# lipku/LiveTalking

Hardware: NVIDIA H100
Metric: lip-sync frames/sec (wav2lip256, 256x256, batch 16, mel + U-Net fwd + paste-back) (higher is better)
Workload: dtype f16 (fp32 accumulate); mel f64; paste u8

## Files before the change

### livetalking_b200/csrc/conv_halo.cu

```cuda
#include <cuda.h>

#include <atomic>
#include <mutex>
#include <utility>

#include "conv_halo.h"
#include "ltb_internal.h"
#include "ptx_sm90.cuh"

#ifdef LTB_HALO_DIAG
#include <cstdlib>
#define LTB_DIAG(bit) (p.dbg & (bit))
#else
#define LTB_DIAG(bit) 0
#endif

namespace ltb {

constexpr int kHaloP = 10;
constexpr int kHaloThreads = 384;
constexpr int kProducerRegs = 40, kConsumerRegs = 232;
constexpr int kSms = 132;

template <int BN, int NSUB, int NACC, int TAPS, int RC = 0>
// ... 478 lines not shown
          const size_t opix = halo_pix(img, ty, tx, q >> 1, 0, wq * 16 + (lane >> 2) + 8 * (q & 1), row_ok);
          if (q < 2 * NSUB && row_ok) {
            float ha0 = head_sw[96], ha1 = head_sw[97], ha2 = head_sw[98];
#pragma unroll
            for (int i = 0; i < 4; ++i)
#pragma unroll
              for (int src = 0; src < 4; ++src) {
                const float2 f = __half22float2(*reinterpret_cast<__half2*>(&hv[src][i]));
                const int cc = 8 * i + 2 * src;
                ha0 = fmaf(f.x, head_sw[cc], ha0);
                ha0 = fmaf(f.y, head_sw[cc + 1], ha0);
                ha1 = fmaf(f.x, head_sw[32 + cc], ha1);
                ha1 = fmaf(f.y, head_sw[32 + cc + 1], ha1);
                ha2 = fmaf(f.x, head_sw[64 + cc], ha2);
                ha2 = fmaf(f.y, head_sw[64 + cc + 1], ha2);
              }
            float* o = p.head_out + opix * 3;
            o[0] = (1.f / (1.f + expf(-ha0))) * 255.f;
            o[1] = (1.f / (1.f + expf(-ha1))) * 255.f;
            o[2] = (1.f / (1.f + expf(-ha2))) * 255.f;
          }
        }
      }
    }
  }

  __syncthreads();
  if (gn_smem) {
    for (int i = tid; i < p.gn_images * p.gn_groups * 2; i += kHaloThreads) {
      const float v = gn_acc[i];
      if (v != 0.f) atomicAdd(p.gn_stats + i, v);
    }
  }
}

typedef CUresult (*EncodeTiledFn)(CUtensorMap*, CUtensorMapDataType, cuuint32_t, void*, const cuuint64_t*, const cuuint64_t*,
                                  const cuuint32_t*, const cuuint32_t*, CUtensorMapInterleave, CUtensorMapSwizzle,
                                  CUtensorMapL2promotion, CUtensorMapFloatOOBfill);

static EncodeTiledFn get_encode() {
  static EncodeTiledFn fn = nullptr;
  static std::once_flag once;
  std::call_once(once, []() {
    void* p = nullptr;
    cudaDriverEntryPointQueryResult q;
    if (cudaGetDriverEntryPoint("cuTensorMapEncodeTiled", &p, cudaEnableDefault, &q) == cudaSuccess &&
        q == cudaDriverEntryPointSuccess)
      fn = reinterpret_cast<EncodeTiledFn>(p);
  });
  return fn;
}

bool encode_tmap_f16(CUtensorMap* tm, int rank, const void* base, const cuuint64_t* dims, const cuuint64_t* strides_bytes,
                     const cuuint32_t* box, int spatial_stride) {
  EncodeTiledFn fn = get_encode();
  if (!fn) return false;
  cuuint32_t es[5] = {1, (cuuint32_t)spatial_stride, (cuuint32_t)spatial_stride, 1, 1};
  return fn(tm, CU_TENSOR_MAP_DATA_TYPE_FLOAT16, (cuuint32_t)rank, const_cast<void*>(base), dims, strides_bytes, box, es,
            CU_TENSOR_MAP_INTERLEAVE_NONE, CU_TENSOR_MAP_SWIZZLE_128B, CU_TENSOR_MAP_L2_PROMOTION_L2_256B,
            CU_TENSOR_MAP_FLOAT_OOB_FILL_NONE) == CUDA_SUCCESS;
}

static bool is_conv3x3(const ConvParams& p) {
  if (p.nphases != 1 || p.ph[0].ntaps != 9 || p.sy != 1 || p.sx != 1 || p.osy != 1 || p.osx != 1) return false;
  for (int t = 0; t < 9; ++t)
    if (p.ph[0].dy[t] != t / 3 - 1 || p.ph[0].dx[t] != t % 3 - 1) return false;
  return p.IH == p.GH && p.IW == p.GW && p.OH == p.GH && p.OW == p.GW;
}
static bool is_convT(const ConvParams& p) {
  if (p.nphases != 4 || p.osy != 2 || p.osx != 2 || p.sy != 1 || p.sx != 1) return false;
  const int nt[4] = {1, 2, 2, 4};
  for (int i = 0; i < 4; ++i)
    if (p.ph[i].ntaps != nt[i]) return false;
  return p.IH == p.GH && p.IW == p.GW && p.OH == 2 * p.GH && p.OW == 2 * p.GW;
}

static bool is_conv3x3_s2(const ConvParams& p) {
  if (p.nphases != 1 || p.ph[0].ntaps != 9 || p.sy != 2 || p.sx != 2 || p.osy != 1 || p.osx != 1) return false;
  for (int t = 0; t < 9; ++t)
    if (p.ph[0].dy[t] != t / 3 - 1 || p.ph[0].dx[t] != t % 3 - 1) return false;
  return p.IH == 2 * p.GH && p.IW == 2 * p.GW && p.OH == p.GH && p.OW == p.GW;
}

static bool is_upconv(const ConvParams& p) {
  return p.upconv == 1 && p.nphases == 4 && p.osy == 2 && p.osx == 2 && p.sy == 1 && p.sx == 1 && p.IH == p.GH && p.IW == p.GW &&
         p.OH == 2 * p.GH && p.OW == 2 * p.GW;
}

static bool is_gemm(const ConvParams& p) {
  return p.nphases == 1 && p.ph[0].ntaps == 1 && p.ph[0].dy[0] == 0 && p.ph[0].dx[0] == 0 && p.sy == 1 && p.sx == 1 && p.osy == 1 &&
         p.osx == 1 && p.IH == p.GH && p.IW == p.GW && p.OH == p.GH && p.OW == p.GW;
}

static bool pick_cfg(const ConvParams& p, int* BN, int* NSUB, int* NACC);

bool conv_halo_supported(const ConvParams& p) {
  if (p.zbatch > 1) return false;
  if ((p.OCtot % 8) || (p.oc_off % 8) || (reinterpret_cast<uintptr_t>(p.out) % 16)) return false;
  if (p.res && ((p.RCtot % 8) || (p.rc_off % 8) || (reinterpret_cast<uintptr_t>(p.res) % 16))) return false;
  if (p.group_slot && (!is_gemm(p) || (p.w_slot_stride * 2) % 16 != 0)) return false;
  if (is_gemm(p)) {
    return p.Cout % 32 == 0 && p.Cin % 8 == 0 && p.Cin >= 32 && (p.ICtot % 8) == 0 && (p.ic_off % 8) == 0 && (p.Ktot % 8) == 0 &&
           (p.ph[0].koff % 8) == 0 && p.M >= 512 && get_encode() != nullptr;
  }
  if (is_conv3x3_s2(p)) {
    return p.Cout % 32 == 0 && p.Cin >= 64 && (p.ICtot % 8) == 0 && (p.ic_off % 8) == 0 && p.Ktot == 9 * p.Cin && p.GH >= 16 &&
           p.GW >= 8 && get_encode() != nullptr;
  }
  if (is_upconv(p))
    return p.Cout % 64 == 0 && p.Cin >= 16 && (p.ICtot % 8) == 0 && (p.ic_off % 8) == 0 && p.Ktot == 16 * p.Cin && get_encode() != nullptr;
  if (!(is_conv3x3(p) || is_convT(p))) return false;
  if (p.Cout % 32 != 0 || p.Cin < 16) return false;
// ... 288 lines not shown
```

### livetalking_b200/csrc/conv_halo.h

```cpp
#pragma once
#include <cuda.h>
#include <cuda_runtime.h>

#include <cstring>

#include "conv_params.h"

namespace ltb {

struct alignas(64) HaloParams {
  CUtensorMap tm_in;
  CUtensorMap tm_w;
  __half* out;
  const __half* res;
  const float* bias;
  int N, M, Cin;
  int OCtot, oc_off, RCtot, rc_off;
  int OH, OW, osy, osx;
  int GH, GW;
  int relu;
  int res_halo;
  int halo_y0, halo_x0;
  int acc_oy[4], acc_ox[4];
  int tiles_x, tiles_y, tiles_n, total_tiles;
  float* gn_stats;
  int gn_groups, gn_cpg, gn_hw, gn_images;
  const float* head_w;
  const float* head_b;
  float* head_out;
  const int* group_slot;
  int group_rows, group_tiles;
  long long bias_slot_stride;
#ifdef LTB_HALO_DIAG
  int dbg;
#endif
};

struct HaloPlan {
  HaloParams hp;
  int BN, NSUB, NACC, TAPS;
  bool grouped;
};

bool conv_halo_supported(const ConvParams& p);
int conv_halo_make_plan(const ConvParams& p, const __half* w_tap_major, HaloPlan* out);
cudaError_t launch_conv_halo(const HaloPlan& pl, cudaStream_t st);
bool encode_tmap_f16(CUtensorMap* tm, int rank, const void* base, const cuuint64_t* dims, const cuuint64_t* strides_bytes,
                     const cuuint32_t* box, int spatial_stride = 1);
int conv_halo_sms();
int conv_halo_resident_chunks(const HaloPlan& pl, int sms);
bool conv_halo_gn_fusable(const HaloPlan& pl, int cout_total, int groups, int hw);
cudaError_t launch_w_tap_major(const __half* w, __half* wt, int cout, int cin, cudaStream_t st, int ntaps = 9);
cudaError_t launch_w_tap_major_convT(const __half* w, __half* wt, int cout, int cin, cudaStream_t st);

}
```

### livetalking_b200/csrc/conv_plan.cu

```cuda
#include <cstring>
#include <string>
#include <vector>

#include "../../include/ltb200.h"
#include "conv_plan.h"
#include "ltb_internal.h"

namespace ltb {

static const int kTd[2][2] = {{0, 0}, {0, 1}};
static const int kTk[2][2] = {{1, 0}, {2, 0}};
static const int kTn[2] = {1, 2};
static const int kUd[2][2] = {{-1, 0}, {0, 1}};

ConvParams conv_params(ConvMode mode, int N, ConvSlice in, int IH, int IW, int Cin, ConvSlice out, int OH, int OW, int Cout,
                       ConvSlice res, const __half* w, int Ktot, int w_koff, const float* bias, bool relu, ConvTaps taps) {
  ConvParams p;
  std::memset(&p, 0, sizeof(p));
  p.in = in.p;
  p.N = N;
  p.IH = IH;
  p.IW = IW;
  p.ICtot = in.Ctot;
  p.ic_off = in.off;
// ... 9 lines not shown
  p.res = res.p;
  p.RCtot = res.Ctot;
  p.rc_off = res.off;
  p.w = w;
  p.Ktot = Ktot;
  p.bias = bias;
  p.relu = relu ? 1 : 0;
  if (mode == ConvMode::Dense) {
    p.sy = taps.sy;
    p.sx = taps.sx;
    p.GH = OH;
    p.GW = OW;
    p.nphases = 1;
    ConvPhase& ph = p.ph[0];
    ph.ntaps = taps.KH * taps.KW;
    ph.koff = w_koff;
    for (int kh = 0; kh < taps.KH; ++kh)
      for (int kw = 0; kw < taps.KW; ++kw) {
        ph.dy[kh * taps.KW + kw] = (signed char)(kh - taps.pad_t);
        ph.dx[kh * taps.KW + kw] = (signed char)(kw - taps.pad_l);
      }
  } else {
    const bool up = mode == ConvMode::Upsample2x;
    p.GH = IH;
    p.GW = IW;
    p.osy = p.osx = 2;
    p.nphases = 4;
    p.upconv = up ? 1 : 0;
    int koff = w_koff;
    for (int a = 0; a < 2; ++a)
      for (int b = 0; b < 2; ++b) {
        ConvPhase& ph = p.ph[a * 2 + b];
        const int na = up ? 2 : kTn[a], nb = up ? 2 : kTn[b];
        ph.ntaps = na * nb;
        ph.koff = koff;
        ph.ooy = a;
        ph.oox = b;
        for (int i = 0; i < na; ++i)
          for (int j = 0; j < nb; ++j) {
            ph.dy[i * nb + j] = (signed char)(up ? kUd[a][i] : kTd[a][i]);
            ph.dx[i * nb + j] = (signed char)(up ? kUd[b][j] : kTd[b][j]);
          }
        koff += ph.ntaps * Cin;
      }
  }
  p.M = N * p.GH * p.GW;
  return p;
}

int conv_plan(const ConvParams& p, const __half* w_tap, ConvPath path, ConvPlan* out) {
  out->p = p;
  out->halo = false;
  out->pingpong = false;
  if (p.group_slot) {
    if (p.group_images < 1 || p.N % p.group_images || p.slots < 1 || p.w_slot_stride < 0 || p.bias_slot_stride < 0)
      return LTB_FAIL("conv: grouped weights need N divisible by group_images >= 1, slots >= 1 and non-negative slot strides");
    if (p.zbatch > 1 || p.upconv) return LTB_FAIL("conv: grouped weights cannot be combined with zbatch or the fused upsample");
  }
  if (path == ConvPath::Gather) return 0;
  if (w_tap && conv_pingpong_supported(p)) {
    if (conv_pingpong_make_plan(p, w_tap, &out->pp) != 0) return LTB_FAIL("conv: ping-pong plan / tensor map creation failed");
    out->pingpong = true;
    return 0;
  }
  const bool gemm = p.nphases == 1 && p.ph[0].ntaps == 1;
  if (!((w_tap || gemm) && conv_halo_supported(p))) {
    if (path == ConvPath::Auto) return 0;
    return LTB_FAIL("conv: the halo kernel cannot run " + std::to_string(p.N) + "x" + std::to_string(p.IH) + "x" + std::to_string(p.IW) +
                    "x" + std::to_string(p.Cin) + " -> " + std::to_string(p.OH) + "x" + std::to_string(p.OW) + "x" + std::to_string(p.Cout) +
                    (w_tap || gemm ? "" : " without tap-major weights"));
  }
  if (conv_halo_make_plan(p, w_tap, &out->hp) != 0) return LTB_FAIL("conv: halo plan / tensor map creation failed");
  out->halo = true;
  return 0;
}

cudaError_t conv_launch(const ConvPlan& pl, cudaStream_t st, float* splitk_ws, size_t ws_floats) {
  if (pl.pingpong) return launch_conv_pingpong(pl.pp, st);
  return pl.halo ? launch_conv_halo(pl.hp, st) : launch_conv_gather(pl.p, st, splitk_ws, ws_floats);
}

bool conv_plan_variant(const ConvPlan& pl, bool have_ws, size_t ws_floats, ltb_conv_variant* out) {
  std::memset(out, 0, sizeof(*out));
  out->grouped = pl.p.group_slot != nullptr;
  if (pl.pingpong) {
    out->kernel = 2;
    out->taps = 9;
    out->bn = 64;
    out->nsub = 1;
    out->nacc = 1;
    out->resident_chunks = 1;
    out->res_halo = 1;
    return true;
  }
  if (pl.halo) {
    out->kernel = 1;
    out->taps = pl.hp.TAPS;
    out->bn = pl.hp.BN;
    out->nsub = pl.hp.NSUB;
    out->nacc = pl.hp.NACC;
    out->resident_chunks = conv_halo_resident_chunks(pl.hp, conv_halo_sms());
    out->res_halo = pl.hp.hp.res_halo;
    return true;
  }
  int ksplit = 0;
  if (!conv_gather_pick(pl.p, have_ws, ws_floats, &out->bn, &out->kb, &ksplit)) return false;
  out->ksplit = ksplit > 1 ? ksplit : 1;
  return true;
}

bool conv_plan_fuse_gn_stats(ConvPlan* pl, float* stats, int groups, int hw) {
  const ConvParams& p = pl->p;
  if (!pl->halo || pl->hp.grouped || p.oc_off != 0 || p.OCtot != p.Cout || !conv_halo_gn_fusable(pl->hp, p.Cout, groups, hw)) return false;
  HaloParams& h = pl->hp.hp;
  h.gn_stats = stats;
  h.gn_groups = groups;
  h.gn_cpg = p.Cout / groups;
  h.gn_hw = hw;
  h.gn_images = p.M / hw;
  return true;
}

bool conv_plan_fuse_head(ConvPlan* pl, const float* w, const float* b, float* out) {
  if (!pl->halo || pl->hp.grouped || pl->hp.BN != 32 || pl->p.Cout != 32) return false;
  pl->hp.hp.head_w = w;
  pl->hp.hp.head_b = b;
  pl->hp.hp.head_out = out;
  return true;
}

static void pack_conv_w(const float* w, int cout, int cin, int KH, int KW, std::vector<__half>& out) {
  out.resize((size_t)cout * KH * KW * cin);
  for (int co = 0; co < cout; ++co)
    for (int kh = 0; kh < KH; ++kh)
      for (int kw = 0; kw < KW; ++kw)
        for (int ci = 0; ci < cin; ++ci)
          out[((size_t)co * KH * KW + kh * KW + kw) * cin + ci] = __float2half(w[(((size_t)co * cin + ci) * KH + kh) * KW + kw]);
}
static void pack_convT_w(const float* w, int cin, int cout, std::vector<__half>& out) {
  out.resize((size_t)cout * 9 * cin);
  for (int co = 0; co < cout; ++co) {
    size_t k = 0;
    for (int a = 0; a < 2; ++a)
      for (int b = 0; b < 2; ++b)
        for (int i = 0; i < kTn[a]; ++i)
          for (int j = 0; j < kTn[b]; ++j) {
            const int kh = kTk[a][i], kw = kTk[b][j];
            for (int ci = 0; ci < cin; ++ci, ++k)
              out[(size_t)co * 9 * cin + k] = __float2half(w[(((size_t)ci * cout + co) * 3 + kh) * 3 + kw]);
          }
  }
}

}

using namespace ltb;

static int conv2d_f16_impl(const ltb_conv_desc* d, const void* in_f16, const float* w_f32, const float* bias_f32,
                           const void* res_f16, void* out_f16, int reps, float* ms_out) {
  if (!d || !in_f16 || !w_f32 || !bias_f32 || !out_f16) return LTB_FAIL("null argument");
  if (d->has_res && !res_f16) return LTB_FAIL("has_res set but res is null");
  int OH, OW, Ktot;
  std::vector<__half> wp;
  if (d->transposed) {
    if (d->KH != 3 || d->KW != 3) return LTB_FAIL("transposed conv: only k=3,s=2,p=1,op=1");
    OH = d->IH * 2;
    OW = d->IW * 2;
    Ktot = 9 * d->Cin;
    pack_convT_w(w_f32, d->Cin, d->Cout, wp);
  } else {
    if (d->KH * d->KW > kMaxTaps) return LTB_FAIL("kernel too large");
    OH = conv_out_dim(d->IH, d->KH, d->sy, d->pad);
    OW = conv_out_dim(d->IW, d->KW, d->sx, d->pad);
    Ktot = d->KH * d->KW * d->Cin;
    pack_conv_w(w_f32, d->Cout, d->Cin, d->KH, d->KW, wp);
  }
  if (OH <= 0 || OW <= 0) return LTB_FAIL("empty output");
  const size_t in_b = (size_t)d->N * d->IH * d->IW * d->Cin * 2, out_b = (size_t)d->N * OH * OW * d->Cout * 2;
  __half *din = nullptr, *dout = nullptr, *dw = nullptr, *dres = nullptr, *dwt = nullptr;
  float* dbias = nullptr;
  float* dws = nullptr;
  cudaEvent_t e0 = nullptr, e1 = nullptr;
  int rc = 0;
  auto cleanup = [&]() {
    cudaFree(din);
    cudaFree(dout);
    cudaFree(dw);
    cudaFree(dres);
    cudaFree(dwt);
    cudaFree(dws);
    cudaFree(dbias);
    if (e0) cudaEventDestroy(e0);
    if (e1) cudaEventDestroy(e1);
  };
#define CK(x)                                                             \
  do {                                                                    \
    cudaError_t _e = (x);                                                 \
    if (_e != cudaSuccess) {                                              \
      rc = LTB_FAIL(std::string(#x) + ": " + cudaGetErrorString(_e));     \
      cleanup();                                                          \
      return rc;                                                          \
    }                                                                     \
  } while (0)
  CK(cudaMalloc(&din, in_b));
  CK(cudaMalloc(&dout, out_b));
  CK(cudaMalloc(&dw, wp.size() * 2));
  CK(cudaMalloc(&dbias, (size_t)d->Cout * 4));
  CK(cudaMemcpy(din, in_f16, in_b, cudaMemcpyHostToDevice));
  CK(cudaMemcpy(dw, wp.data(), wp.size() * 2, cudaMemcpyHostToDevice));
  CK(cudaMemcpy(dbias, bias_f32, (size_t)d->Cout * 4, cudaMemcpyHostToDevice));
  CK(cudaMemset(dout, 0xFF, out_b));
  if (d->has_res) {
    CK(cudaMalloc(&dres, out_b));
    CK(cudaMemcpy(dres, res_f16, out_b, cudaMemcpyHostToDevice));
  }
  if (d->KH == 3 && d->KW == 3) {
    CK(cudaMalloc(&dwt, wp.size() * 2));
    CK(d->transposed ? launch_w_tap_major_convT(dw, dwt, d->Cout, d->Cin, nullptr) : launch_w_tap_major(dw, dwt, d->Cout, d->Cin, nullptr));
  }
  const ConvParams p = conv_params(d->transposed ? ConvMode::Transposed : ConvMode::Dense, d->N, {din, d->Cin, 0}, d->IH, d->IW, d->Cin,
                                   {dout, d->Cout, 0}, OH, OW, d->Cout, d->has_res ? ConvSlice{dres, d->Cout, 0} : ConvSlice{}, dw, Ktot, 0,
                                   dbias, d->relu != 0, {d->KH, d->KW, d->sy, d->sx, d->pad, d->pad});
  const ConvPath path = d->force_path == 1 ? ConvPath::Gather : d->force_path == 2 ? ConvPath::Halo : ConvPath::Auto;
  ConvPlan pl;
  if (conv_plan(p, dwt, path, &pl)) {
    cleanup();
    return 1;
  }
  const size_t ws_floats = (pl.halo || pl.pingpong) ? 0 : (size_t)1 << 22;
  if (ws_floats) {
    CK(cudaMalloc(&dws, ws_floats * sizeof(float)));
    CK(cudaMemset(dws, 0, ws_floats * sizeof(float)));
  }
  CK(conv_launch(pl, nullptr, dws, ws_floats));
  if (reps > 0) {
    CK(cudaEventCreate(&e0));
    CK(cudaEventCreate(&e1));
    for (int i = 0; i < 3; ++i) CK(conv_launch(pl, nullptr, dws, ws_floats));
    CK(cudaEventRecord(e0, nullptr));
    for (int i = 0; i < reps; ++i) CK(conv_launch(pl, nullptr, dws, ws_floats));
    CK(cudaEventRecord(e1, nullptr));
    CK(cudaEventSynchronize(e1));
    CK(cudaEventElapsedTime(ms_out, e0, e1));
    *ms_out /= reps;
  }
  CK(cudaDeviceSynchronize());
  CK(cudaMemcpy(out_f16, dout, out_b, cudaMemcpyDeviceToHost));
#undef CK
  cleanup();
  return 0;
}

extern "C" {

int ltb_conv2d_f16(const ltb_conv_desc* d, const void* in_f16, const float* w_f32, const float* bias_f32,
                   const void* res_f16, void* out_f16) {
  return conv2d_f16_impl(d, in_f16, w_f32, bias_f32, res_f16, out_f16, 0, nullptr);
}

int ltb_conv2d_f16_timed(const ltb_conv_desc* d, const void* in_f16, const float* w_f32, const float* bias_f32,
                         const void* res_f16, void* out_f16, int reps, float* ms_per_launch) {
  if (reps < 1 || !ms_per_launch) return LTB_FAIL("conv2d_f16_timed: reps >= 1 and a result pointer are required");
  return conv2d_f16_impl(d, in_f16, w_f32, bias_f32, res_f16, out_f16, reps, ms_per_launch);
}

}
```

### livetalking_b200/csrc/conv_plan.h

```cpp
#pragma once
#include <cuda_runtime.h>

#include "conv_halo.h"
#include "conv_pingpong.h"

struct ltb_conv_variant;

namespace ltb {

struct ConvSlice {
  const __half* p;
  int Ctot, off;
};

enum class ConvMode {
  Dense,
  Transposed,
  Upsample2x,
};
struct ConvTaps {
  int KH, KW, sy, sx, pad_t, pad_l;
};

inline int conv_out_dim(int in, int k, int s, int pad) { return (in + 2 * pad - k) / s + 1; }

ConvParams conv_params(ConvMode mode, int N, ConvSlice in, int IH, int IW, int Cin, ConvSlice out, int OH, int OW, int Cout,
                       ConvSlice res, const __half* w, int Ktot, int w_koff, const float* bias, bool relu, ConvTaps taps = {});

enum class ConvPath {
  Auto,
  Gather,
  Halo,
};
struct ConvPlan {
  ConvParams p{};
  bool halo = false;
  HaloPlan hp{};
  bool pingpong = false;
  PingpongParams pp{};
};

int conv_plan(const ConvParams& p, const __half* w_tap, ConvPath path, ConvPlan* out);
cudaError_t conv_launch(const ConvPlan& pl, cudaStream_t st, float* splitk_ws, size_t ws_floats);
bool conv_plan_variant(const ConvPlan& pl, bool have_ws, size_t ws_floats, ltb_conv_variant* out);

bool conv_plan_fuse_gn_stats(ConvPlan* pl, float* stats, int groups, int hw);
bool conv_plan_fuse_head(ConvPlan* pl, const float* w, const float* b, float* out);

}
```

### livetalking_b200/csrc/ptx_sm90.cuh

```cuda
#pragma once
#include <cuda_fp16.h>
#include <cstdint>
#include <cstdio>

namespace ltb {

__device__ __forceinline__ uint32_t smem_u32(const void* p) {
  return static_cast<uint32_t>(__cvta_generic_to_shared(p));
}

__device__ __forceinline__ void mbar_init(uint32_t bar, uint32_t count) {
  asm volatile("mbarrier.init.shared::cta.b64 [%0], %1;" ::"r"(bar), "r"(count) : "memory");
}
__device__ __forceinline__ void mbar_fence_init() {
  asm volatile("fence.mbarrier_init.release.cluster;" ::: "memory");
}
__device__ __forceinline__ void mbar_arrive(uint32_t bar) {
  asm volatile("mbarrier.arrive.shared::cta.b64 _, [%0];" ::"r"(bar) : "memory");
}
__device__ __forceinline__ void mbar_arrive_expect_tx(uint32_t bar, uint32_t bytes) {
  asm volatile("mbarrier.arrive.expect_tx.shared::cta.b64 _, [%0], %1;" ::"r"(bar), "r"(bytes) : "memory");
}
__device__ __forceinline__ bool mbar_try_wait(uint32_t bar, uint32_t parity) {
  uint32_t ok;
// ... 62 lines not shown
      "l"(tmap), "r"(bar), "r"(c0), "r"(c1), "r"(c2), "r"(c3), "r"(c4)
      : "memory");
}

__device__ __forceinline__ void ldmatrix_x4(uint32_t& r0, uint32_t& r1, uint32_t& r2, uint32_t& r3, uint32_t saddr) {
  asm volatile("ldmatrix.sync.aligned.m8n8.x4.shared.b16 {%0, %1, %2, %3}, [%4];"
               : "=r"(r0), "=r"(r1), "=r"(r2), "=r"(r3)
               : "r"(saddr)
               : "memory");
}

__device__ __forceinline__ void ldmatrix_x4_trans(uint32_t& r0, uint32_t& r1, uint32_t& r2, uint32_t& r3, uint32_t saddr) {
  asm volatile("ldmatrix.sync.aligned.m8n8.x4.trans.shared.b16 {%0, %1, %2, %3}, [%4];"
               : "=r"(r0), "=r"(r1), "=r"(r2), "=r"(r3)
               : "r"(saddr)
               : "memory");
}
__device__ __forceinline__ void stmatrix_x4_trans(uint32_t saddr, uint32_t r0, uint32_t r1, uint32_t r2, uint32_t r3) {
  asm volatile("stmatrix.sync.aligned.m8n8.x4.trans.shared.b16 [%0], {%1, %2, %3, %4};" ::"r"(saddr), "r"(r0), "r"(r1), "r"(r2), "r"(r3)
               : "memory");
}

__device__ __forceinline__ void tma_store_4d(const void* tmap, uint32_t src, int c0, int c1, int c2, int c3) {
  asm volatile("cp.async.bulk.tensor.4d.global.shared::cta.bulk_group [%0, {%2, %3, %4, %5}], [%1];" ::"l"(tmap), "r"(src), "r"(c0),
               "r"(c1), "r"(c2), "r"(c3)
               : "memory");
}
__device__ __forceinline__ void bulk_commit() { asm volatile("cp.async.bulk.commit_group;" ::: "memory"); }
template <int N>
__device__ __forceinline__ void bulk_wait_read() {
  asm volatile("cp.async.bulk.wait_group.read %0;" ::"n"(N) : "memory");
}
template <int N>
__device__ __forceinline__ void bulk_wait() {
  asm volatile("cp.async.bulk.wait_group %0;" ::"n"(N) : "memory");
}

__device__ __forceinline__ void named_sync(uint32_t id, uint32_t threads) {
  asm volatile("bar.sync %0, %1;" ::"r"(id), "r"(threads) : "memory");
}
__device__ __forceinline__ void named_arrive(uint32_t id, uint32_t threads) {
  asm volatile("bar.arrive %0, %1;" ::"r"(id), "r"(threads) : "memory");
}

__device__ __forceinline__ uint64_t wgmma_desc(uint32_t saddr, uint32_t lbo_bytes, uint32_t sbo_bytes, uint32_t layout) {
  uint64_t d = 0;
  d |= (uint64_t)((saddr & 0x3FFFF) >> 4);
  d |= (uint64_t)((lbo_bytes >> 4) & 0x3FFF) << 16;
  d |= (uint64_t)((sbo_bytes >> 4) & 0x3FFF) << 32;
  d |= (uint64_t)(layout & 3) << 62;
  return d;
}
__host__ __device__ constexpr uint32_t wgmma_hi_128b(uint32_t sbo_bytes) { return (sbo_bytes >> 4) | (1u << 30); }
__device__ __forceinline__ uint32_t wgmma_lo(uint32_t saddr) { return ((saddr & 0x3FFFFu) >> 4) | (1u << 16); }
__device__ __forceinline__ uint64_t wgmma_lohi(uint32_t lo, uint32_t hi) { return ((uint64_t)hi << 32) | lo; }

__device__ __forceinline__ void wgmma_fence() { asm volatile("wgmma.fence.sync.aligned;" ::: "memory"); }
__device__ __forceinline__ void wgmma_commit() { asm volatile("wgmma.commit_group.sync.aligned;" ::: "memory"); }
template <int N>
__device__ __forceinline__ void wgmma_wait() {
  asm volatile("wgmma.wait_group.sync.aligned %0;" ::"n"(N) : "memory");
}
template <int R>
__device__ __forceinline__ void wgmma_fence_regs(float (&d)[R]) {
#pragma unroll
  for (int i = 0; i < R; ++i) asm volatile("" : "+f"(d[i])::"memory");
}

template <int N>
struct Wgmma;
#define LTB_D1(i) "+f"(d[i])
#define LTB_D2(i) LTB_D1(i), LTB_D1(i + 1)
#define LTB_D4(i) LTB_D2(i), LTB_D2(i + 2)
#define LTB_D8(i) LTB_D4(i), LTB_D4(i + 4)
#define LTB_D16(i) LTB_D8(i), LTB_D8(i + 8)
#define LTB_D32(i) LTB_D16(i), LTB_D16(i + 16)
#define LTB_D64(i) LTB_D32(i), LTB_D32(i + 32)
#define LTB_D128(i) LTB_D64(i), LTB_D64(i + 64)
#define LTB_WG_HEAD(P) "{\n.reg .pred p;\nsetp.ne.b32 p, %" P ", 0;\nwgmma.mma_async.sync.aligned.m64n"
#define LTB_WG_SS(N, REGS, A, B, P) LTB_WG_HEAD(P) N "k16.f32.f16.f16 " REGS ", %" A ", %" B ", p, 1, 1, 0, 0;\n}\n"
#define LTB_WG_RS(N, REGS, A, B, P) \
  LTB_WG_HEAD(P) N "k16.f32.f16.f16 " REGS ", {%" A "}, %" B ", p, 1, 1, 0;\n}\n"

template <>
struct Wgmma<16> {
#define LTB_R "{%0,%1,%2,%3,%4,%5,%6,%7}"
  __device__ __forceinline__ static void ss(float (&d)[8], uint64_t a, uint64_t b, uint32_t acc) {
    asm volatile(LTB_WG_SS("16", LTB_R, "8", "9", "10") : LTB_D8(0) : "l"(a), "l"(b), "r"(acc));
  }
  __device__ __forceinline__ static void rs(float (&d)[8], const uint32_t (&a)[4], uint64_t b, uint32_t acc) {
    asm volatile(LTB_WG_RS("16", LTB_R, "8,%9,%10,%11", "12", "13") : LTB_D8(0)
                 : "r"(a[0]), "r"(a[1]), "r"(a[2]), "r"(a[3]), "l"(b), "r"(acc));
  }
#undef LTB_R
};

template <>
struct Wgmma<32> {
#define LTB_R "{%0,%1,%2,%3,%4,%5,%6,%7,%8,%9,%10,%11,%12,%13,%14,%15}"
  __device__ __forceinline__ static void ss(float (&d)[16], uint64_t a, uint64_t b, uint32_t acc) {
    asm volatile(LTB_WG_SS("32", LTB_R, "16", "17", "18") : LTB_D16(0) : "l"(a), "l"(b), "r"(acc));
  }
  __device__ __forceinline__ static void rs(float (&d)[16], const uint32_t (&a)[4], uint64_t b, uint32_t acc) {
    asm volatile(LTB_WG_RS("32", LTB_R, "16,%17,%18,%19", "20", "21") : LTB_D16(0)
                 : "r"(a[0]), "r"(a[1]), "r"(a[2]), "r"(a[3]), "l"(b), "r"(acc));
  }
// ... 151 lines not shown
```

### livetalking_b200/csrc/w2l_engine.cu

```cuda
#include <cstring>
#include <memory>
#include <mutex>
#include <string>
#include <vector>

#include "../../include/ltb200.h"
#include "conv_plan.h"
#include "ltb_internal.h"
#include "stem_umma.h"

namespace ltb {

static thread_local std::string g_last_error;
void set_error(const std::string& msg) { g_last_error = msg; }

bool pdl_default() {
  static const bool on = [] {
    const char* e = std::getenv("LTB_NO_PDL");
    return !(e && e[0] && e[0] != '0');
  }();
  return on;
}
static thread_local int g_pdl = -1;
bool pdl_enabled() { return g_pdl < 0 ? pdl_default() : g_pdl == 1; }
// ... 240 lines not shown
  const int catS[8] = {512, 512, 512, 256, 128, 64, 32, 16};
  __half* cat[8];
  for (int i = 0; i < 8; ++i) {
    void* p;
    if (dev_alloc(s, (size_t)B * catH[i] * catH[i] * (catD[i] + catS[i]) * 2, &p, true)) return 1;
    cat[i] = static_cast<__half*>(p);
  }
  const size_t tmp_bytes = (size_t)B * 256 * 256 * 64 * 2;
  __half* ring[2] = {nullptr, nullptr};
  int ring_next = 0;
  auto new_tmp = [&](int H, int W, int C, View* v) -> int {
    void* p = nullptr;
    if (keep) {
      if (dev_alloc(s, (size_t)B * H * W * C * 2, &p, true)) return 1;
    } else {
      if (!ring[ring_next]) {
        if (dev_alloc(s, tmp_bytes, &p, true)) return 1;
        ring[ring_next] = static_cast<__half*>(p);
      }
      p = ring[ring_next];
      ring_next ^= 1;
    }
    *v = View{static_cast<__half*>(p), H, W, C, 0, C};
    return 0;
  };
  __half* aring[2] = {nullptr, nullptr};
  int aring_next = 0;
  auto new_atmp = [&](int H, int W, int C, View* v) -> int {
    void* p = nullptr;
    if (keep) {
      if (dev_alloc(s, (size_t)B * H * W * C * 2, &p, true)) return 1;
    } else {
      if (!aring[aring_next]) {
        if (dev_alloc(s, (size_t)B * 80 * 16 * 32 * 2, &p, true)) return 1;
        aring[aring_next] = static_cast<__half*>(p);
      }
      p = aring[aring_next];
      aring_next ^= 1;
    }
    *v = View{static_cast<__half*>(p), H, W, C, 0, C};
    return 0;
  };
  auto cat_dec = [&](int i) { return View{cat[i], catH[i], catH[i], catD[i] + catS[i], 0, catD[i]}; };
  auto cat_skip = [&](int i) { return View{cat[i], catH[i], catH[i], catD[i] + catS[i], catD[i], catS[i]}; };
  auto cat_all = [&](int i) { return View{cat[i], catH[i], catH[i], catD[i] + catS[i], 0, catD[i] + catS[i]}; };

  auto record = [&](int li, const View& v) {
    s->louts[li] = LayerOut{v.p, v.H, v.W, v.C, v.Ctot, v.c_off};
  };
  const ConvPath path = (s->flags & LTB_SESSION_NO_HALO) ? ConvPath::Gather : ConvPath::Auto;
  auto push_conv = [&](int li, const ConvParams& p) -> int {
    Op o;
    if (conv_plan(p, m->wt[li], path, &o.conv)) return LTB_FAIL("plan: layer " + std::to_string(li) + ": " + g_last_error);
    o.type = (o.conv.halo || o.conv.pingpong) ? 4 : 0;
    s->ops.push_back(o);
    return 0;
  };
  auto add_conv = [&](int li, const View& in, const View& out, const View* res) -> int {
    const LDef& L = kLayers[li];
    if (in.C != L.cin || out.C != L.cout) return LTB_FAIL("plan: channel mismatch at layer " + std::to_string(li));
    const int OH = conv_out_dim(in.H, L.k, L.sy, L.pad), OW = conv_out_dim(in.W, L.k, L.sx, L.pad);
    if (OH != out.H || OW != out.W) return LTB_FAIL("plan: spatial mismatch at layer " + std::to_string(li));
    const ConvParams p = conv_params(ConvMode::Dense, B, in.slice(), in.H, in.W, L.cin, out.slice(), OH, OW, L.cout,
                                     res ? res->slice() : ConvSlice{}, m->w[li], L.k * L.k * L.cin, 0, m->bias[li], true,
                                     {L.k, L.k, L.sy, L.sx, L.pad, L.pad});
    if (push_conv(li, p)) return 1;
    record(li, out);
    return 0;
  };
  auto add_convT = [&](int li, const View& in, const View& out) -> int {
    const LDef& L = kLayers[li];
    if (in.C != L.cin || out.C != L.cout || out.H != 2 * in.H) return LTB_FAIL("plan: convT mismatch at layer " + std::to_string(li));
    const ConvParams p = conv_params(ConvMode::Transposed, B, in.slice(), in.H, in.W, L.cin, out.slice(), out.H, out.W, L.cout,
                                     ConvSlice{}, m->w[li], 9 * L.cin, 0, m->bias[li], true);
    if (push_conv(li, p)) return 1;
    record(li, out);
    return 0;
  };

  {
    Op o;
    o.type = 6;
    o.branch = 1;
    s->ops.push_back(o);
  }
  View a_prev;
  if (new_atmp(80, 16, 32, &a_prev)) return 1;
  {
    Op o;
    o.type = 2;
    o.audio_out = a_prev.p;
    o.branch = 1;
    s->ops.push_back(o);
    record(0, a_prev);
  }
  {
    int H = 80, W = 16;
    for (int li = 1; li <= 12; ++li) {
      const LDef& L = kLayers[li];
      const int OH = conv_out_dim(H, L.k, L.sy, L.pad), OW = conv_out_dim(W, L.k, L.sx, L.pad);
      View o;
      if (new_atmp(OH, OW, L.cout, &o)) return 1;
      if (add_conv(li, a_prev, o, L.res ? &a_prev : nullptr)) return 1;
      s->ops.back().branch = 1;
      a_prev = o;
      H = OH;
      W = OW;
// ... 750 lines not shown
```

Measured before the change: 7362.

## Add row-pair WGMMA kernel for final 80-to-32 channel 3x3 conv with fused head

Adds a specialized warp-specialized TMA+WGMMA kernel for 3x3 stride-1 convolutions with 80 input and 32 output channels, tiling 32 rows by 8 columns. Output pixels are treated as the wide N dimension, and a 64+16 channel split uses 128B and 32B swizzled tensor maps. The kernel can fuse the RGB sigmoid head. Two consumer warpgroups alternate tiles with ordered WGMMA issue, aiming to improve tensor core utilisation on the large full-resolution last layers over the generic halo kernel. It adds a new code path gated by an environment variable and tile count, and its numerical correctness depends on the descriptor layouts.

New measurement: 7583, median of 6. +3.0%, better.

```diff
diff --git a/livetalking_b200/csrc/conv_halo.cu b/livetalking_b200/csrc/conv_halo.cu
--- a/livetalking_b200/csrc/conv_halo.cu
+++ b/livetalking_b200/csrc/conv_halo.cu
@@ -554,12 +554,12 @@
 }
 
 bool encode_tmap_f16(CUtensorMap* tm, int rank, const void* base, const cuuint64_t* dims, const cuuint64_t* strides_bytes,
-                     const cuuint32_t* box, int spatial_stride) {
+                     const cuuint32_t* box, int spatial_stride, CUtensorMapSwizzle swizzle) {
   EncodeTiledFn fn = get_encode();
   if (!fn) return false;
   cuuint32_t es[5] = {1, (cuuint32_t)spatial_stride, (cuuint32_t)spatial_stride, 1, 1};
   return fn(tm, CU_TENSOR_MAP_DATA_TYPE_FLOAT16, (cuuint32_t)rank, const_cast<void*>(base), dims, strides_bytes, box, es,
-            CU_TENSOR_MAP_INTERLEAVE_NONE, CU_TENSOR_MAP_SWIZZLE_128B, CU_TENSOR_MAP_L2_PROMOTION_L2_256B,
+            CU_TENSOR_MAP_INTERLEAVE_NONE, swizzle, CU_TENSOR_MAP_L2_PROMOTION_L2_256B,
             CU_TENSOR_MAP_FLOAT_OOB_FILL_NONE) == CUDA_SUCCESS;
 }
 
diff --git a/livetalking_b200/csrc/conv_halo.h b/livetalking_b200/csrc/conv_halo.h
--- a/livetalking_b200/csrc/conv_halo.h
+++ b/livetalking_b200/csrc/conv_halo.h
@@ -46,7 +46,7 @@
 int conv_halo_make_plan(const ConvParams& p, const __half* w_tap_major, HaloPlan* out);
 cudaError_t launch_conv_halo(const HaloPlan& pl, cudaStream_t st);
 bool encode_tmap_f16(CUtensorMap* tm, int rank, const void* base, const cuuint64_t* dims, const cuuint64_t* strides_bytes,
-                     const cuuint32_t* box, int spatial_stride = 1);
+                     const cuuint32_t* box, int spatial_stride = 1, CUtensorMapSwizzle swizzle = CU_TENSOR_MAP_SWIZZLE_128B);
 int conv_halo_sms();
 int conv_halo_resident_chunks(const HaloPlan& pl, int sms);
 bool conv_halo_gn_fusable(const HaloPlan& pl, int cout_total, int groups, int hw);
diff --git a/livetalking_b200/csrc/conv_plan.cu b/livetalking_b200/csrc/conv_plan.cu
--- a/livetalking_b200/csrc/conv_plan.cu
+++ b/livetalking_b200/csrc/conv_plan.cu
@@ -85,6 +85,7 @@
   out->p = p;
   out->halo = false;
   out->pingpong = false;
+  out->rowpair = false;
   if (p.group_slot) {
     if (p.group_images < 1 || p.N % p.group_images || p.slots < 1 || p.w_slot_stride < 0 || p.bias_slot_stride < 0)
       return LTB_FAIL("conv: grouped weights need N divisible by group_images >= 1, slots >= 1 and non-negative slot strides");
@@ -94,6 +95,11 @@
   if (w_tap && conv_pingpong_supported(p)) {
     if (conv_pingpong_make_plan(p, w_tap, &out->pp) != 0) return LTB_FAIL("conv: ping-pong plan / tensor map creation failed");
     out->pingpong = true;
+    return 0;
+  }
+  if (w_tap && conv_rowpair_supported(p)) {
+    if (conv_rowpair_make_plan(p, w_tap, &out->rp) != 0) return LTB_FAIL("conv: row-pair plan / tensor map creation failed");
+    out->rowpair = true;
     return 0;
   }
   const bool gemm = p.nphases == 1 && p.ph[0].ntaps == 1;
@@ -110,6 +116,7 @@
 
 cudaError_t conv_launch(const ConvPlan& pl, cudaStream_t st, float* splitk_ws, size_t ws_floats) {
   if (pl.pingpong) return launch_conv_pingpong(pl.pp, st);
+  if (pl.rowpair) return launch_conv_rowpair(pl.rp, st);
   return pl.halo ? launch_conv_halo(pl.hp, st) : launch_conv_gather(pl.p, st, splitk_ws, ws_floats);
 }
 
@@ -126,6 +133,15 @@
     out->res_halo = 1;
     return true;
   }
+  if (pl.rowpair) {
+    out->kernel = 3;
+    out->taps = 9;
+    out->bn = 32;
+    out->nsub = 1;
+    out->nacc = 1;
+    out->resident_chunks = 2;
+    return true;
+  }
   if (pl.halo) {
     out->kernel = 1;
     out->taps = pl.hp.TAPS;
@@ -155,6 +171,12 @@
 }
 
 bool conv_plan_fuse_head(ConvPlan* pl, const float* w, const float* b, float* out) {
+  if (pl->rowpair) {
+    pl->rp.head_w = w;
+    pl->rp.head_b = b;
+    pl->rp.head_out = out;
+    return true;
+  }
   if (!pl->halo || pl->hp.grouped || pl->hp.BN != 32 || pl->p.Cout != 32) return false;
   pl->hp.hp.head_w = w;
   pl->hp.hp.head_b = b;
@@ -260,7 +282,7 @@
     cleanup();
     return 1;
   }
-  const size_t ws_floats = (pl.halo || pl.pingpong) ? 0 : (size_t)1 << 22;
+  const size_t ws_floats = (pl.halo || pl.pingpong || pl.rowpair) ? 0 : (size_t)1 << 22;
   if (ws_floats) {
     CK(cudaMalloc(&dws, ws_floats * sizeof(float)));
     CK(cudaMemset(dws, 0, ws_floats * sizeof(float)));
diff --git a/livetalking_b200/csrc/conv_plan.h b/livetalking_b200/csrc/conv_plan.h
--- a/livetalking_b200/csrc/conv_plan.h
+++ b/livetalking_b200/csrc/conv_plan.h
@@ -3,6 +3,7 @@
 
 #include "conv_halo.h"
 #include "conv_pingpong.h"
+#include "conv_rowpair.h"
 
 struct ltb_conv_variant;
 
@@ -38,6 +39,8 @@
   HaloPlan hp{};
   bool pingpong = false;
   PingpongParams pp{};
+  bool rowpair = false;
+  RowpairParams rp{};
 };
 
 int conv_plan(const ConvParams& p, const __half* w_tap, ConvPath path, ConvPlan* out);
diff --git a/livetalking_b200/csrc/conv_rowpair.cu b/livetalking_b200/csrc/conv_rowpair.cu
--- /dev/null
+++ b/livetalking_b200/csrc/conv_rowpair.cu
@@ -0,0 +1,265 @@
+#include <cuda.h>
+
+#include <cstdlib>
+#include <cstring>
+
+#include "conv_halo.h"
+#include "conv_rowpair.h"
+#include "ltb_internal.h"
+#include "ptx_sm90.cuh"
+
+namespace ltb {
+
+namespace {
+
+constexpr int kThreads = 384;
+constexpr int kProducerRegs = 40, kConsumerRegs = 232;
+constexpr int kTH = 32;
+constexpr int kN = 4 * kTH;
+constexpr int kP = 10, kHR = kTH + 2;
+constexpr int kStages = 2;
+constexpr int kX0Raw = kHR * kP * 128;
+constexpr int kX1Raw = kHR * kP * 32;
+constexpr int kX0Bytes = (kX0Raw + 1023) & ~1023;
+constexpr int kX1Bytes = (kX1Raw + 1023) & ~1023;
+constexpr int kStageBytes = kX0Bytes + kX1Bytes;
+constexpr int kBlk0 = 32 * 128, kBlk1 = 32 * 32;
+constexpr int kBlocks = 13;
+constexpr int kW0Bytes = kBlocks * kBlk0, kW1Bytes = kBlocks * kBlk1;
+constexpr int kWTxBytes = 9 * (kBlk0 + kBlk1);
+constexpr int kOutBytes = kTH * 8 * 64;
+constexpr int kSmemBytes = kW0Bytes + kW1Bytes + kStages * kStageBytes + 2 * kOutBytes + 1024;
+static_assert(kSmemBytes + 1024 <= 227 * 1024, "shared memory overflow");
+constexpr uint32_t kBarOrder = 1, kBarStage = 3;
+
+}
+
+__global__ void __launch_bounds__(kThreads, 1) conv_rowpair_kernel(const __grid_constant__ RowpairParams p) {
+  extern __shared__ uint8_t smem_raw[];
+  __shared__ __align__(8) uint64_t x_full[kStages], x_empty[kStages], w_full;
+  __shared__ float head_sw[99];
+  const int tid = threadIdx.x, warp = tid >> 5, lane = tid & 31;
+  const uint32_t smem0 = (smem_u32(smem_raw) + 1023u) & ~1023u;
+  uint8_t* const smem = smem_raw + (smem0 - smem_u32(smem_raw));
+  const uint32_t w0_smem = smem0;
+  const uint32_t w1_smem = w0_smem + kW0Bytes;
+  const uint32_t x_smem = w1_smem + kW1Bytes;
+  const uint32_t o_smem = x_smem + kStages * kStageBytes;
+  const int tiles_img = p.tiles_x * p.tiles_y;
+
+  for (int i = tid; i < 4 * (kBlk0 + kBlk1) / 16; i += kThreads) {
+    const int z = i / ((kBlk0 + kBlk1) / 16), r = i - z * ((kBlk0 + kBlk1) / 16);
+    const int off = r < kBlk0 / 16 ? 4 * z * kBlk0 + r * 16 : kW0Bytes + 4 * z * kBlk1 + (r - kBlk0 / 16) * 16;
+    *reinterpret_cast<uint4*>(smem + off) = make_uint4(0u, 0u, 0u, 0u);
+  }
+  fence_proxy_async_smem();
+  if (p.head_out && tid < 99) head_sw[tid] = (tid < 96) ? p.head_w[tid] : p.head_b[tid - 96];
+  if (tid == 0) {
+    for (int s = 0; s < kStages; ++s) {
+      mbar_init(smem_u32(&x_full[s]), 1);
+      mbar_init(smem_u32(&x_empty[s]), 4);
+    }
+    mbar_init(smem_u32(&w_full), 1);
+    mbar_fence_init();
+    tma_prefetch_desc(&p.tm_x0);
+    tma_prefetch_desc(&p.tm_x1);
+    tma_prefetch_desc(&p.tm_w0);
+    tma_prefetch_desc(&p.tm_w1);
+    tma_prefetch_desc(&p.tm_out);
+  }
+  __syncthreads();
+
+  pdl_launch_dependents();
+  if (warp == 8 && lane == 0) {
+    mbar_arrive_expect_tx(smem_u32(&w_full), kWTxBytes);
+    for (int t = 0; t < 9; ++t) {
+      const int b = 4 * (t % 3) + 3 - t / 3;
+      tma_load_3d(w0_smem + b * kBlk0, &p.tm_w0, smem_u32(&w_full), 0, 0, t);
+      tma_load_3d(w1_smem + b * kBlk1, &p.tm_w1, smem_u32(&w_full), 64, 0, t);
+    }
+  }
+  pdl_wait();
+
+  if (warp >= 8) {
+    setmaxnreg_dec<kProducerRegs>();
+    if (warp == 8 && lane == 0) {
+      uint32_t s = 0;
+      for (int t = blockIdx.x; t < p.total_tiles; t += gridDim.x, ++s) {
+        const int img = t / tiles_img, r = t - img * tiles_img;
+        const int ty = r / p.tiles_x, tx = r - ty * p.tiles_x;
+        const uint32_t st = s % kStages;
+        const uint32_t xb = x_smem + st * kStageBytes;
+        mbar_wait(smem_u32(&x_empty[st]), ((s / kStages) & 1u) ^ 1u);
+        mbar_arrive_expect_tx(smem_u32(&x_full[st]), kX0Raw + kX1Raw);
+        tma_load_4d(xb, &p.tm_x0, smem_u32(&x_full[st]), 0, tx * 8 - 1, ty * kTH - 1, img);
+        tma_load_4d(xb + kX0Bytes, &p.tm_x1, smem_u32(&x_full[st]), 64, tx * 8 - 1, ty * kTH - 1, img);
+      }
+    }
+    return;
+  }
+
+  setmaxnreg_inc<kConsumerRegs>();
+  const int wg = warp >> 2, wq = warp & 3;
+  const bool leader = (tid & 127) == 0;
+  const bool head = p.head_out != nullptr;
+  const uint32_t obuf = o_smem + wg * kOutBytes;
+  constexpr uint32_t kW0Hi = wgmma_hi_128b(8 * 128);
+  constexpr uint32_t kW1Hi = wgmma_hi_32b(8 * 32);
+  constexpr uint32_t kX0Hi = wgmma_hi_128b(2 * kP * 128);
+  constexpr uint32_t kX1Hi = wgmma_hi_32b(2 * kP * 32);
+  const uint32_t w0_lo = wgmma_lo(w0_smem), w1_lo = wgmma_lo(w1_smem);
+  const int par = wq >> 1, c0 = 16 * (wq & 1) + (lane >> 2);
+  const float bias0 = __ldg(p.bias + c0), bias1 = __ldg(p.bias + c0 + 8);
+  const int sm_i = lane >> 4, sm_cb = 2 * (wq & 1) + ((lane >> 3) & 1), sm_x = lane & 7;
+  const uint32_t sm_off = (uint32_t)(sm_x * 64 + ((sm_cb ^ ((sm_x >> 1) & 3)) << 4));
+  mbar_wait(smem_u32(&w_full), 0);
+
+  uint32_t s = wg;
+  for (int t = blockIdx.x + wg * gridDim.x; t < p.total_tiles; t += 2 * gridDim.x, s += 2) {
+    const int img = t / tiles_img, r = t - img * tiles_img;
+    const int ty = r / p.tiles_x, tx = r - ty * p.tiles_x;
+    const uint32_t st = s % kStages;
+    const uint32_t xb = x_smem + st * kStageBytes;
+    if (s > 0) named_sync(kBarOrder + wg, 256);
+    mbar_wait(smem_u32(&x_full[st]), (s / kStages) & 1u);
+
+    float acc[kN / 2];
+#pragma unroll
+    for (int i = 0; i < kN / 2; ++i) acc[i] = 0.f;
+    const uint32_t x0_lo = wgmma_lo(xb), x1_lo = wgmma_lo(xb + kX0Bytes);
+    wgmma_fence();
+#pragma unroll
+    for (int v = 0; v < 4; ++v)
+#pragma unroll
+      for (int k = 0; k < 4; ++k)
+#pragma unroll
+        for (int dx = 0; dx < 3; ++dx)
+          Wgmma<kN>::ss(acc, wgmma_lohi(w0_lo + (4 * dx + 3 - v) * (kBlk0 / 16) + k * 2, kW0Hi),
+                        wgmma_lohi(x0_lo + (v * kP + dx) * 8 + k * 2, kX0Hi), 1u);
+#pragma unroll
+    for (int v = 0; v < 4; ++v)
+#pragma unroll
+      for (int dx = 0; dx < 3; ++dx)
+        Wgmma<kN>::ss(acc, wgmma_lohi(w1_lo + (4 * dx + 3 - v) * (kBlk1 / 16), kW1Hi), wgmma_lohi(x1_lo + (v * kP + dx) * 2, kX1Hi), 1u);
+    wgmma_commit();
+    if (t + gridDim.x < p.total_tiles) named_arrive(kBarOrder + (wg ^ 1), 256);
+    wgmma_wait<0>();
+    wgmma_fence_regs(acc);
+    __syncwarp();
+    if (lane == 0) mbar_arrive(smem_u32(&x_empty[st]));
+
+    if (leader) bulk_wait_read<0>();
+    named_sync(kBarStage + wg, 128);
+    auto cvt = [&](float f0, float f1, float b) { return p.relu ? f32x2_to_f16x2_sat_relu(f0 + b, f1 + b) : f32x2_to_f16x2_sat(f0 + b, f1 + b); };
+#pragma unroll
+    for (int i = 0; i < kTH / 2; i += 2) {
+      const uint32_t o0 = cvt(acc[4 * i], acc[4 * i + 1], bias0);
+      const uint32_t o1 = cvt(acc[4 * i + 2], acc[4 * i + 3], bias1);
+      const uint32_t o2 = cvt(acc[4 * i + 4], acc[4 * i + 5], bias0);
+      const uint32_t o3 = cvt(acc[4 * i + 6], acc[4 * i + 7], bias1);
+      stmatrix_x4_trans(obuf + (2 * (i + sm_i) + par) * 8 * 64 + sm_off, o0, o1, o2, o3);
+    }
+    if (!head) fence_proxy_async_smem();
+    named_sync(kBarStage + wg, 128);
+    if (!head) {
+      if (leader) {
+        tma_store_4d(&p.tm_out, obuf, 0, tx * 8, ty * kTH, img);
+        bulk_commit();
+      }
+      continue;
+    }
+#pragma unroll 1
+    for (int pix = tid & 127; pix < kTH * 8; pix += 128) {
+      const int gy = ty * kTH + (pix >> 3), gx = tx * 8 + (pix & 7);
+      if (gy >= p.H || gx >= p.W) continue;
+      uint32_t hv[16];
+#pragma unroll
+      for (int cb = 0; cb < 4; ++cb) {
+        const uint4 q = lds128(obuf + pix * 64 + ((cb ^ ((pix >> 1) & 3)) << 4));
+        hv[4 * cb] = q.x;
+        hv[4 * cb + 1] = q.y;
+        hv[4 * cb + 2] = q.z;
+        hv[4 * cb + 3] = q.w;
+      }
+      float ha0 = head_sw[96], ha1 = head_sw[97], ha2 = head_sw[98];
+#pragma unroll
+      for (int j = 0; j < 16; ++j) {
+        const float2 f = __half22float2(*reinterpret_cast<const __half2*>(&hv[j]));
+        ha0 = fmaf(f.x, head_sw[2 * j], ha0);
+        ha0 = fmaf(f.y, head_sw[2 * j + 1], ha0);
+        ha1 = fmaf(f.x, head_sw[32 + 2 * j], ha1);
+        ha1 = fmaf(f.y, head_sw[32 + 2 * j + 1], ha1);
+        ha2 = fmaf(f.x, head_sw[64 + 2 * j], ha2);
+        ha2 = fmaf(f.y, head_sw[64 + 2 * j + 1], ha2);
+      }
+      float* o = p.head_out + (((size_t)img * p.H + gy) * p.W + gx) * 3;
+      o[0] = (1.f / (1.f + expf(-ha0))) * 255.f;
+      o[1] = (1.f / (1.f + expf(-ha1))) * 255.f;
+      o[2] = (1.f / (1.f + expf(-ha2))) * 255.f;
+    }
+  }
+  if (leader) bulk_wait<0>();
+}
+
+static bool rowpair_enabled() {
+  const char* e = std::getenv("LTB_CONV_ROWPAIR");
+  return !(e && std::strcmp(e, "0") == 0);
+}
+
+bool conv_rowpair_supported(const ConvParams& p) {
+  if (p.zbatch > 1 || p.group_slot || p.upconv || p.nphases != 1 || p.ph[0].ntaps != 9) return false;
+  if (p.sy != 1 || p.sx != 1 || p.osy != 1 || p.osx != 1) return false;
+  for (int t = 0; t < 9; ++t)
+    if (p.ph[0].dy[t] != t / 3 - 1 || p.ph[0].dx[t] != t % 3 - 1) return false;
+  if (p.IH != p.GH || p.IW != p.GW || p.OH != p.GH || p.OW != p.GW) return false;
+  if (p.Cin != 80 || p.Cout != 32 || p.Ktot != 9 * 80 || p.res) return false;
+  if ((p.ICtot % 8) || (p.ic_off % 8) || (p.OCtot % 8) || (p.oc_off % 8) || (reinterpret_cast<uintptr_t>(p.out) % 16) ||
+      (reinterpret_cast<uintptr_t>(p.in) % 16))
+    return false;
+  const long tiles = (long)p.N * ((p.GH + kTH - 1) / kTH) * ((p.GW + 7) / 8);
+  if (tiles < 3L * conv_halo_sms()) return false;
+  return rowpair_enabled();
+}
+
+int conv_rowpair_make_plan(const ConvParams& p, const __half* w_tap_major, RowpairParams* out) {
+  if (!conv_rowpair_supported(p) || !w_tap_major) return 1;
+  std::memset(out, 0, sizeof(*out));
+  {
+    const cuuint64_t dims[4] = {(cuuint64_t)p.Cin, (cuuint64_t)p.IW, (cuuint64_t)p.IH, (cuuint64_t)p.N};
+    const cuuint64_t strides[3] = {(cuuint64_t)p.ICtot * 2, (cuuint64_t)p.IW * p.ICtot * 2, (cuuint64_t)p.IH * p.IW * p.ICtot * 2};
+    const cuuint32_t box0[4] = {64, kP, kHR, 1}, box1[4] = {16, kP, kHR, 1};
+    if (!encode_tmap_f16(&out->tm_x0, 4, p.in + p.ic_off, dims, strides, box0)) return 2;
+    if (!encode_tmap_f16(&out->tm_x1, 4, p.in + p.ic_off, dims, strides, box1, 1, CU_TENSOR_MAP_SWIZZLE_32B)) return 2;
+  }
+  {
+    const cuuint64_t dims[3] = {(cuuint64_t)p.Cin, 32, 9};
+    const cuuint64_t strides[2] = {(cuuint64_t)p.Cin * 2, (cuuint64_t)32 * p.Cin * 2};
+    const cuuint32_t box0[3] = {64, 32, 1}, box1[3] = {16, 32, 1};
+    if (!encode_tmap_f16(&out->tm_w0, 3, w_tap_major, dims, strides, box0)) return 2;
+    if (!encode_tmap_f16(&out->tm_w1, 3, w_tap_major, dims, strides, box1, 1, CU_TENSOR_MAP_SWIZZLE_32B)) return 2;
+  }
+  {
+    const cuuint64_t dims[4] = {32, (cuuint64_t)p.OW, (cuuint64_t)p.OH, (cuuint64_t)p.N};
+    const cuuint64_t strides[3] = {(cuuint64_t)p.OCtot * 2, (cuuint64_t)p.OW * p.OCtot * 2, (cuuint64_t)p.OH * p.OW * p.OCtot * 2};
+    const cuuint32_t box[4] = {32, 8, kTH, 1};
+    if (!encode_tmap_f16(&out->tm_out, 4, p.out + p.oc_off, dims, strides, box, 1, CU_TENSOR_MAP_SWIZZLE_64B)) return 2;
+  }
+  out->bias = p.bias;
+  out->relu = p.relu;
+  out->H = p.GH;
+  out->W = p.GW;
+  out->tiles_x = (p.GW + 7) / 8;
+  out->tiles_y = (p.GH + kTH - 1) / kTH;
+  out->total_tiles = out->tiles_x * out->tiles_y * p.N;
+  return 0;
+}
+
+cudaError_t launch_conv_rowpair(const RowpairParams& rp, cudaStream_t st) {
+  static SmemConfigOnce once;
+  if (cudaError_t e = once.ensure(conv_rowpair_kernel, kSmemBytes); e != cudaSuccess) return e;
+  const int sms = conv_halo_sms();
+  const int grid = rp.total_tiles < sms ? rp.total_tiles : sms;
+  return launch_kernel_pdl(conv_rowpair_kernel, dim3(grid), dim3(kThreads), kSmemBytes, st, rp);
+}
+
+}
diff --git a/livetalking_b200/csrc/conv_rowpair.h b/livetalking_b200/csrc/conv_rowpair.h
--- /dev/null
+++ b/livetalking_b200/csrc/conv_rowpair.h
@@ -0,0 +1,28 @@
+#pragma once
+#include <cuda.h>
+#include <cuda_runtime.h>
+
+#include "conv_params.h"
+
+namespace ltb {
+
+struct alignas(64) RowpairParams {
+  CUtensorMap tm_x0;
+  CUtensorMap tm_x1;
+  CUtensorMap tm_w0;
+  CUtensorMap tm_w1;
+  CUtensorMap tm_out;
+  const float* bias;
+  const float* head_w;
+  const float* head_b;
+  float* head_out;
+  int relu;
+  int H, W;
+  int tiles_x, tiles_y, total_tiles;
+};
+
+bool conv_rowpair_supported(const ConvParams& p);
+int conv_rowpair_make_plan(const ConvParams& p, const __half* w_tap_major, RowpairParams* out);
+cudaError_t launch_conv_rowpair(const RowpairParams& rp, cudaStream_t st);
+
+}
diff --git a/livetalking_b200/csrc/ptx_sm90.cuh b/livetalking_b200/csrc/ptx_sm90.cuh
--- a/livetalking_b200/csrc/ptx_sm90.cuh
+++ b/livetalking_b200/csrc/ptx_sm90.cuh
@@ -138,6 +138,7 @@
   return d;
 }
 __host__ __device__ constexpr uint32_t wgmma_hi_128b(uint32_t sbo_bytes) { return (sbo_bytes >> 4) | (1u << 30); }
+__host__ __device__ constexpr uint32_t wgmma_hi_32b(uint32_t sbo_bytes) { return (sbo_bytes >> 4) | (3u << 30); }
 __device__ __forceinline__ uint32_t wgmma_lo(uint32_t saddr) { return ((saddr & 0x3FFFFu) >> 4) | (1u << 16); }
 __device__ __forceinline__ uint64_t wgmma_lohi(uint32_t lo, uint32_t hi) { return ((uint64_t)hi << 32) | lo; }
 
diff --git a/livetalking_b200/csrc/w2l_engine.cu b/livetalking_b200/csrc/w2l_engine.cu
--- a/livetalking_b200/csrc/w2l_engine.cu
+++ b/livetalking_b200/csrc/w2l_engine.cu
@@ -316,7 +316,7 @@
   auto push_conv = [&](int li, const ConvParams& p) -> int {
     Op o;
     if (conv_plan(p, m->wt[li], path, &o.conv)) return LTB_FAIL("plan: layer " + std::to_string(li) + ": " + g_last_error);
-    o.type = (o.conv.halo || o.conv.pingpong) ? 4 : 0;
+    o.type = (o.conv.halo || o.conv.pingpong || o.conv.rowpair) ? 4 : 0;
     s->ops.push_back(o);
     return 0;
   };
```
